# dwofk/fast-depth

Hardware: NVIDIA H100
Metric: depth-maps/sec @224x224 b64 (higher is better)
Workload: dtype f16

## Files before the change

fastdepth_b200/csrc/fd_block_tc.cu:

```cuda
#include <cuda.h>

#include <cstdio>
#include <cstdlib>
#include <cstring>
#include <new>
#include <string>

#include "fd_block_plan.h"
#include "fd_tc_common.cuh"

namespace fd {

constexpr int TC_DW_WARPS = 8;
constexpr int TC_EPI_WARPS = 8;
constexpr int TC_WARP_EPI0 = 0, TC_WARP_DW0 = TC_EPI_WARPS;
constexpr int TC_WARP_TMA = TC_DW_WARPS + TC_EPI_WARPS;
constexpr int TC_THREADS = (TC_WARP_TMA + 1) * 32;
constexpr int TC_WARP_BCAST = TC_WARP_TMA + 1;
constexpr int TC_THREADS_CL = (TC_WARP_BCAST + 1) * 32;
constexpr int TC_NCH = 2;
constexpr int TC_KBLK = 64;
constexpr int TC_A_STAGE_BYTES = 128 * 128;
constexpr int TC_MAX_IN = 6, TC_MAX_A = 6, TC_MAX_B = 16;
static_assert(TC_MAX_A >= kPlanMaxACluster && TC_MAX_A >= kPlanMaxA && TC_MAX_IN >= kPlanMaxIn && TC_MAX_B >= kPlanMaxB, "barrier arrays cover the planner's ring depths");
constexpr int TC_TRACE_N = 256;

struct TcParams {
    int n, h_in, w_in, h_out, w_out, c_in, c_out;
    int tiles_x, tiles_y;
    int items, splits;
    int kblocks;
    int cin_pad;
    int n_cta;
    int bn;
// ... 44 lines not shown
    const int split = w - (int)t * p.splits;
    uint32_t t2 = fdiv40(t, p.mg_tx);
    const int tile_x = (int)(t - t2 * (uint32_t)p.tiles_x);
    uint32_t t3 = fdiv40(t2, p.mg_ty);
    const int tile_y = (int)(t2 - t3 * (uint32_t)p.tiles_y);
    c.img0 = (int)t3 * NI; c.oy0 = tile_y * TH; c.ox0 = tile_x * TW; c.n0 = split * p.n_cta;
    return c;
}

#define TC_TRACE(row, idx)                                                                       \
    do {                                                                                         \
        if (p.trace != nullptr && blockIdx.x == 0 && (idx) < TC_TRACE_N) p.trace[(row) * TC_TRACE_N + (idx)] = clock64(); \
    } while (0)

template <typename T, int KS, int STRIDE, int NI, int TH, int TW, bool RELU6, bool HALFK = false, int CLM = 0>
__global__ void __launch_bounds__(CLM == 1 ? TC_THREADS_CL : TC_THREADS, 1)
block_tc_kernel(const __grid_constant__ CUtensorMap tm_in, const __grid_constant__ CUtensorMap tm_w,
                const __grid_constant__ CUtensorMap tm_o0, const __grid_constant__ CUtensorMap tm_o1,
                const __grid_constant__ CUtensorMap tm_o2, const __grid_constant__ CUtensorMap tm_o3, const TcParams p) {
    static_assert(NI * TH * TW == 128, "tile must hold 128 pixels");
    static_assert(NI * (TH / 4) * (TW / 4) == TC_DW_WARPS, "one 4x4 pixel block per depthwise warp");
    constexpr int PAD = (KS - 1) / 2;
    constexpr int IH = (TH - 1) * STRIDE + KS, IW = (TW - 1) * STRIDE + KS;
    constexpr int IBH = 3 * STRIDE + KS, IBW = 3 * STRIDE + KS;
    using MF = MixFma<T>;

    extern __shared__ uint8_t smem_raw[];
    const uint32_t smem_base = (smem_u32(smem_raw) + 1023u) & ~1023u;
    uint8_t* smem = smem_raw + (smem_base - smem_u32(smem_raw));
    const uint32_t a_off = 0;
    const uint32_t b_off = a_off + p.s_a * TC_A_STAGE_BYTES;
// ... 45 lines not shown
        tma_prefetch_desc(&tm_w);
        if (p.epi_tma) { tma_prefetch_desc(&tm_o0); if (p.upsample) { tma_prefetch_desc(&tm_o1); tma_prefetch_desc(&tm_o2); tma_prefetch_desc(&tm_o3); } }
    }
    if (p.head)
        for (int i = 2 * threadIdx.x; i < p.cpad_all; i += 2 * (int)blockDim.x) s_head_w2[i >> 1] = MF::pack(p.head_w[i], p.head_w[i + 1]);
    if constexpr (HALFK) {
        for (int i = threadIdx.x; i < p.s_a * (TC_A_STAGE_BYTES / 16); i += (int)blockDim.x)
            reinterpret_cast<uint4*>(smem + a_off)[i] = make_uint4(0u, 0u, 0u, 0u);
        fence_proxy_async();
    }
    pdl_launch_dependents();
    pdl_wait_prior_grid();
    if constexpr (CLM != 0) cluster_sync_all();
    else __syncthreads();

    if (warp == TC_WARP_TMA) {
        if (lane == 0) {
            Ring rin;
            int tr = 0;
            for (int u = u_first; u < u_count; u += u_stride) {
                const int w = item_of(u);
                const ItemCoord c = decode_item(p, w, NI, TH, TW);
                for (int kb = CL ? (int)crank : 0; kb < p.kblocks; kb += (int)cs, rin.next((uint32_t)p.s_in)) {
                    const uint32_t s = rin.s, ph = rin.ph;
                    mbar_wait_sleep_sel<kHint>(smem_u32(&bars->in_empty[s]), ph ^ 1u, (uint32_t)p.sleep_ns >> 2);
                    mbar_expect_tx(smem_u32(&bars->in_full[s]), (uint32_t)(p.in_stage_bytes + p.dwp_bytes));
                    tma_load_4d(smem_base + in_off + s * p.in_stage_stride, &tm_in, smem_u32(&bars->in_full[s]), kb * TC_KBLK,
                                c.ox0 * STRIDE - PAD, c.oy0 * STRIDE - PAD, c.img0);
                    bulk_load(smem_base + in_off + s * p.in_stage_stride + p.in_stage_bytes,
                              reinterpret_cast<const uint8_t*>(p.dwp) + (size_t)kb * p.dwp_bytes, (uint32_t)p.dwp_bytes,
// ... 34 lines not shown
        if (lane == 0) {
            Ring ra;
            uint32_t o = 0;
            for (int u = u_first; u < u_count; u += u_stride)
                for (int kb = 0; kb < p.kblocks; ++kb, ra.next((uint32_t)p.s_a)) {
                    if ((uint32_t)kb % cs != crank) continue;
                    mbar_wait_sel<kHint>(smem_u32(&bars->dw_done[o & 3u]), (o >> 2) & 1u);
                    ++o;
                    const uint32_t slot = smem_base + a_off + ra.s * TC_A_STAGE_BYTES, bar = smem_u32(&bars->a_full[ra.s]);
                    mbar_arrive(bar);
                    for (uint32_t peer = 0; peer < cs; ++peer)
                        if (peer != crank) bulk_copy_to_peer(mapa_u32(slot, peer), slot, (uint32_t)TC_A_STAGE_BYTES, mapa_u32(bar, peer));
                }
        }
    } else if (rwarp >= TC_WARP_DW0 && rwarp < TC_WARP_DW0 + TC_DW_WARPS) {
        constexpr int BPR = TW / 4, BPI = (TH / 4) * BPR;
        const int dwi = rwarp - TC_WARP_DW0;
        const int teams = CL ? 1 : p.dw_teams;
        const int team = teams == 2 ? dwi >> 2 : 0, member = teams == 2 ? dwi & 3 : dwi, nblk = teams;
        Ring rin, ra;
        int tr = 0;
        uint32_t own = 0;
        const bool tracer = dwi == 0 && lane == 0;
        for (int u = u_first; u < u_count; u += u_stride) {
            for (int kb = 0; kb < p.kblocks; ++kb, ra.next((uint32_t)p.s_a)) {
                if (CL && (uint32_t)kb % cs != crank) {
                    mbar_wait_sel<kHint>(smem_u32(&bars->a_empty[ra.s]), ra.ph ^ 1u);
                    continue;
                }
                const uint32_t s = rin.s, ph = rin.ph, sa = ra.s, pha = ra.ph;
                rin.next((uint32_t)p.s_in);
                if (teams == 2 && (int)(own & 1u) != team) { ++own; continue; }
                mbar_wait_sleep_sel<kHint>(smem_u32(&bars->in_full[s]), ph, (uint32_t)p.dw_sleep_ns);
                if (tracer) TC_TRACE(1, tr);
                const uint8_t* stage = smem + in_off + s * p.in_stage_stride;
                const uint8_t* prm = stage + p.in_stage_bytes;
                const f32x2 sc = *reinterpret_cast<const f32x2*>(prm + KS * KS * 128 + lane * 8);
                const f32x2 bi = *reinterpret_cast<const f32x2*>(prm + KS * KS * 128 + 256 + lane * 8);
                mbar_wait_sel<kHint>(smem_u32(&bars->a_empty[sa]), pha ^ 1u);
                uint8_t* a_s = smem + a_off + sa * TC_A_STAGE_BYTES;
                constexpr bool kDwFfma2 = KS == 3;
                uint32_t wv[(HALFK || kDwFfma2) ? 1 : KS * KS];
                if constexpr (!HALFK && !kDwFfma2) {
#pragma unroll
                    for (int i = 0; i < KS * KS; ++i) wv[i] = *reinterpret_cast<const uint32_t*>(prm + i * 128 + lane * 4);
                }
#pragma unroll 1
                for (int blk = 0; blk < nblk; ++blk) {
                const int bidx = member * nblk + blk;
                const int ni = bidx / BPI, rem = bidx % BPI, br = rem / BPR, bc = rem % BPR;
                const uint8_t* in_s = stage + (uint32_t)((ni * IH + br * 4 * STRIDE) * IW + bc * 4 * STRIDE) * 128u + lane * 4u;
                if constexpr (HALFK) {
                    static_assert(KS == 3 && STRIDE == 1, "half-K depthwise exists for the 3x3 stride-1 block only");
                    const int hl = lane & 15, hh = lane >> 4;
                    const uint8_t* in_h = in_s - lane * 4 + hl * 4 + (hh * 2 * IW) * 128;
                    const f32x2 sc2 = *reinterpret_cast<const f32x2*>(prm + KS * KS * 128 + hl * 8);
                    const f32x2 bi2 = *reinterpret_cast<const f32x2*>(prm + KS * KS * 128 + 256 + hl * 8);
                    f32x2 acc[2][4];
#pragma unroll
                    for (int a = 0; a < 2; ++a)
// ... 52 lines not shown
#pragma unroll
                            for (int ox = 0; ox < 4; ++ox)
#pragma unroll
                                for (int kx = 0; kx < KS; ++kx) ffma2(acc[oy][ox], row[ox * STRIDE + kx], wq[ky][kx]);
                            if (ky == KS - 1) {
#pragma unroll
                                for (int ox = 0; ox < 4; ++ox) {
                                    const int m = (ni * TH + br * 4 + oy) * TW + bc * 4 + ox;
                                    *reinterpret_cast<uint32_t*>(a_s + m * 128 + (((lane >> 2) ^ (m & 7)) << 4) + ((lane & 3) << 2)) =
                                        MF::template pack_act<RELU6>(ffma2_abc(acc[oy][ox], sc, bi));
                                }
                            }
                        }
                    }
                } else {
                    float acc[4][4][2];
#pragma unroll
                    for (int a = 0; a < 4; ++a)
#pragma unroll
                        for (int b = 0; b < 4; ++b) acc[a][b][0] = acc[a][b][1] = 0.f;
#pragma unroll
                    for (int iy = 0; iy < IBH; ++iy) {
                        uint32_t row[IBW];
#pragma unroll
                        for (int ix = 0; ix < IBW; ++ix) row[ix] = *reinterpret_cast<const uint32_t*>(in_s + (iy * IW + ix) * 128);
#pragma unroll
                        for (int oy = 0; oy < 4; ++oy) {
                            const int ky = iy - oy * STRIDE;
                            if (ky < 0 || ky >= KS) continue;
#pragma unroll
                            for (int ox = 0; ox < 4; ++ox)
#pragma unroll
                                for (int kx = 0; kx < KS; ++kx)
                                    MF::fma2(acc[oy][ox][0], acc[oy][ox][1], row[ox * STRIDE + kx], wv[ky * KS + kx]);
                            if (ky == KS - 1) {
#pragma unroll
                                for (int ox = 0; ox < 4; ++ox) {
                                    const int m = (ni * TH + br * 4 + oy) * TW + bc * 4 + ox;
                                    *reinterpret_cast<uint32_t*>(a_s + m * 128 + (((lane >> 2) ^ (m & 7)) << 4) + ((lane & 3) << 2)) =
                                        MF::template pack_act<RELU6>(ffma2_abc(f32x2_make(acc[oy][ox][0], acc[oy][ox][1]), sc, bi));
                                }
                            }
                        }
                    }
                }
                }
                if (tracer) TC_TRACE(2, tr);
                __syncwarp();
                if (lane == 0) mbar_arrive(smem_u32(&bars->in_empty[s]));
                fence_proxy_async();
                __syncwarp();
                if (lane == 0) mbar_arrive(CL ? smem_u32(&bars->dw_done[own & 3u]) : smem_u32(&bars->a_full[sa]));
                ++own;
                if (tracer) { TC_TRACE(3, tr); ++tr; }
            }
        }
    } else {
        const int ew = rwarp - TC_WARP_EPI0;
        const int wg = ew >> 2, wq = ew & 3;
        const int r0 = wg * 64 + wq * 16 + (lane >> 2), cq = (lane & 3) * 2;
        const bool leader = wq == 0 && lane == 0;
        const bool elected = ew == 0 && lane == 0;
        constexpr uint32_t bar_id = 1u, bar_n = 256u;
        T* __restrict__ outp = reinterpret_cast<T*>(p.out);
        const T* __restrict__ skipp = reinterpret_cast<const T*>(p.skip);
        const int n_stg = p.n_stg < 2 ? 1 : 2;
        const int nch = (p.n_cta + 63) >> 6;
        const int bn_ch = p.bn >> 6;
        const uint32_t a_lo0 = sw128_desc_lo(smem_base + a_off + (uint32_t)wg * 8192u), b_lo0 = sw128_desc_lo(smem_base + b_off);
        const uint32_t a_step = TC_A_STAGE_BYTES >> 4, b_step = (uint32_t)p.b_stage_bytes >> 4;
        Ring ra, rb;
        int tr = 0;
// ... 29 lines not shown
                        --q_left;
                    }
                }
                if (elected) TC_TRACE(4, tr);
                uint32_t sbs[TC_NCH] = {0u, 0u};
                for (int nbi = 0; nbi * bn_ch < nch; ++nbi) {
                    uint32_t sb;
                    if (p.b_resident) {
                        sb = (uint32_t)(kb * (nch / bn_ch) + nbi);
                        if (first) mbar_wait_sel<kHint>(smem_u32(&bars->b_full[sb]), 0);
                    } else {
                        sb = rb.s;
                        mbar_wait_sel<kHint>(smem_u32(&bars->b_full[sb]), rb.ph);
                        rb.next((uint32_t)p.s_b);
                    }
                    sbs[nbi] = sb;
                }
                const uint32_t a_lo = a_lo0 + ra.s * a_step;
                wgmma_fence();
#pragma unroll
                for (int j = 0; j < TC_NCH; ++j) {
                    if (j < nch) {
                        const uint32_t b_lo = b_lo0 + (bn_ch == 2 ? sbs[0] * b_step + (uint32_t)j * 512u : sbs[j] * b_step);
#pragma unroll
                        for (int k4 = 0; k4 < 4; ++k4)
                            wgmma_n64<T>(acc[j], sw128_desc(a_lo + 2u * k4), sw128_desc(b_lo + 2u * k4), (kb > 0 || k4 > 0) ? 1u : 0u);
                    }
                }
                wgmma_commit();
                wgmma_wait0();
                if (leader) {
                    const uint32_t bar_a = smem_u32(&bars->a_empty[ra.s]);
                    if constexpr (CL) { for (uint32_t r = 0; r < cs; ++r) mbar_arrive_cluster(mapa_u32(bar_a, r)); }
                    else mbar_arrive(bar_a);
                    if (!p.b_resident)
                        for (int nbi = 0; nbi * bn_ch < nch; ++nbi) {
                            const uint32_t bar_b = smem_u32(&bars->b_empty[sbs[nbi]]);
                            if constexpr (CW) { for (uint32_t r = 0; r < wmc; ++r) mbar_arrive_cluster(mapa_u32(bar_b, r)); }
                            else mbar_arrive(bar_b);
                        }
                }
                if (elected) { TC_TRACE(5, tr); ++tr; }
            }

            if (!p.head) {
                const float2* aff = s_pw_affine + c.n0;
#pragma unroll
                for (int cb = 0; cb < TC_NCH; ++cb) {
                    if (cb >= nch) break;
                    uint8_t* stg = smem + stg_off + (n_stg == 2 ? (stg_flip & 1u) * 16384u : 0u);
                    ++stg_flip;
                    if (n_stg == 1 && stg_flip > 1) {
// ... 176 lines not shown

template <typename T, int KS, int STRIDE, int NI, int TH, int TW, bool RELU6, bool HALFK = false, int CLM = 0>
static int launch_inst2(BlockTcPlan* bp, cudaStream_t st) {
    auto kern = block_tc_kernel<T, KS, STRIDE, NI, TH, TW, RELU6, HALFK, CLM>;
    constexpr bool CL = CLM != 0;
    const int csize = CLM == 1 ? bp->p.cs : bp->p.wmc;
    const int units = CLM == 1 ? bp->tiles : bp->p.items / (bp->p.wmc > 0 ? bp->p.wmc : 1);
    static PerDeviceOnce attr_set;
    int dev = -1;
    FD_CUDA_OK(cudaGetDevice(&dev));
    if (attr_set.need(dev)) {
        FD_CUDA_OK(cudaFuncSetAttribute(kern, cudaFuncAttributeMaxDynamicSharedMemorySize, 227 * 1024));
        attr_set.done(dev);
    }
    cudaLaunchConfig_t cfg{};
    cfg.gridDim = bp->grid; cfg.blockDim = dim3(CLM == 1 ? TC_THREADS_CL : TC_THREADS); cfg.dynamicSmemBytes = bp->smem_bytes; cfg.stream = st;
    cudaLaunchAttribute attr[2];
    int na = 0;
    if (CL) {
        attr[na].id = cudaLaunchAttributeClusterDimension;
        attr[na].val.clusterDim.x = (unsigned)csize; attr[na].val.clusterDim.y = 1; attr[na].val.clusterDim.z = 1;
        ++na;
    }
    if (CL && !bp->grid_final) {
        cfg.attrs = attr; cfg.numAttrs = (unsigned)na;
        cfg.gridDim = dim3((unsigned)(units * csize), 1, 1);
        int n_cl = 0;
        FD_CUDA_OK(cudaOccupancyMaxActiveClusters(&n_cl, kern, &cfg));
        if (n_cl < 1) return fail(FD_ERR_UNSUPPORTED, "cluster-mode block kernel: no cluster of this shape fits the device");
        if (n_cl > units) n_cl = units;
        bp->grid = dim3((unsigned)(n_cl * csize), 1, 1);
// ... 275 lines not shown
```

fastdepth_b200/csrc/fd_chain_tc.cu:

```cuda
#include <cuda.h>

#include <cstdio>
#include <cstdlib>
#include <cstring>
#include <new>
#include <string>
#include <vector>

#include "fd_tc_common.cuh"

namespace fd {

constexpr int CH_WORKERS = 16;
constexpr int CH_WARP_TMA = 16;
constexpr int CH_THREADS = 17 * 32;
constexpr int CH_MAX_PASS = 4;
constexpr int CH_MAX_LAYERS = 8, CH_MAX_KB = 8;
constexpr int CH_PITCH = 15, CH_ROWS = 9;
constexpr int CH_BLK = 136 * 128;
constexpr int CH_IN_BYTES = CH_ROWS * CH_PITCH * 128;
constexpr int CH_SB = 4, CH_B_STAGE = 128 * 128;
constexpr int CH_SD = 4, CH_DWP = 9 * 128 + 512;
constexpr int CH_AFF_BYTES = 512 * 8;
constexpr int CH_OFF_ACT = 1024;
constexpr int CH_OFF_B = CH_OFF_ACT + CH_MAX_KB * CH_BLK;
constexpr int CH_OFF_DWP = CH_OFF_B + CH_SB * CH_B_STAGE;
constexpr int CH_OFF_AFF = CH_OFF_DWP + CH_SD * CH_DWP;
constexpr int CH_OFF_BAR = CH_OFF_AFF + 2 * CH_AFF_BYTES;

struct ChainBarriers {
// ... 25 lines not shown
    int out_pitch;
    int sleep_ns;
    int n_zero[2];
    void* out;
    ChainLayer L[CH_MAX_LAYERS];
    unsigned long long* trace;
    unsigned char zero_slots[2][48];
};

struct ChainMaps {
    CUtensorMap in;
    CUtensorMap w[CH_MAX_LAYERS];
    CUtensorMap out[2];
};

__device__ __forceinline__ void st_cluster_u32(uint32_t cluster_addr, uint32_t v) {
    asm volatile("st.shared::cluster.b32 [%0], %1;" ::"r"(cluster_addr), "r"(v) : "memory");
}

#define CH_TRACE(row, idx)                                                                                \
    do {                                                                                                  \
        if (p.trace != nullptr && blockIdx.x == 0 && (idx) < 256) p.trace[(row) * 256 + (idx)] = clock64(); \
    } while (0)

template <typename T, bool RELU6>
__global__ void __cluster_dims__(2, 1, 1) __launch_bounds__(CH_THREADS, 1)
chain_tc_kernel(const __grid_constant__ ChainMaps maps, const __grid_constant__ ChainParams p) {
    using MF = MixFma<T>;
    extern __shared__ uint8_t smem_raw[];
    const uint32_t smem_base = (smem_u32(smem_raw) + 1023u) & ~1023u;
// ... 14 lines not shown
        mbar_init(smem_u32(&bars->halo_full), 1);
        mbar_init(smem_u32(&bars->act_free), 1);
        fence_barrier_init();
    }
    for (int i = threadIdx.x; i < (CH_OFF_B) / 16; i += CH_THREADS) reinterpret_cast<uint4*>(smem)[i] = make_uint4(0u, 0u, 0u, 0u);
    fence_proxy_async();
    if (warp == CH_WARP_TMA && lane == 0) {
        tma_prefetch_desc(&maps.in);
        tma_prefetch_desc(&maps.out[rank]);
        for (int l = 0; l < p.n_layers; ++l) tma_prefetch_desc(&maps.w[l]);
    }
    pdl_launch_dependents();
    pdl_wait_prior_grid();
    cluster_sync_all();

    if (warp == CH_WARP_TMA) {
        if (lane == 0) {
            uint32_t seq = 0;
            for (int img = cluster_id; img < p.n_img; img += n_clusters)
                for (int l = 0; l < p.n_layers; ++l) {
                    const ChainLayer& L = p.L[l];
                    for (int ps = 0; ps < L.np; ++ps)
                        for (int kb = 0; kb < L.kblocks; ++kb, ++seq) {
                            const uint32_t s = seq & (CH_SB - 1), ph = (seq / CH_SB) & 1u;
                            mbar_wait_sleep(smem_u32(&bars->b_empty[s]), ph ^ 1u, (uint32_t)p.sleep_ns);
                            if (kb == 0 && ps == 0 && img == cluster_id) CH_TRACE(10, l);
                            mbar_expect_tx(smem_u32(&bars->b_full[s]), (uint32_t)CH_B_STAGE);
                            tma_load_2d(smem_base + CH_OFF_B + s * CH_B_STAGE, &maps.w[l], smem_u32(&bars->b_full[s]), kb * 64, ps * 128);
                        }
                }
        } else if (lane == 1) {
            uint32_t dseq = 0, lseq = 0;
// ... 13 lines not shown
                        bulk_load(smem_base + CH_OFF_DWP + s * CH_DWP, reinterpret_cast<const uint8_t*>(L.dwp) + (size_t)kb * CH_DWP,
                                  (uint32_t)CH_DWP, smem_u32(&bars->dwp_full[s]));
                    }
                }
        } else if (lane == 2) {
            uint32_t it = 0;
            for (int img = cluster_id; img < p.n_img; img += n_clusters, ++it) {
                if (it > 0) mbar_wait_sleep(smem_u32(&bars->act_free), (it - 1u) & 1u, (uint32_t)p.sleep_ns);
                for (int kb = 0; kb < p.L[0].kblocks; ++kb) {
                    mbar_expect_tx(smem_u32(&bars->in_full[kb]), (uint32_t)CH_IN_BYTES);
                    tma_load_4d(smem_base + CH_OFF_ACT + kb * CH_BLK, &maps.in, smem_u32(&bars->in_full[kb]), kb * 64, 0, row_first - 1, img);
                }
            }
        }
    } else {
        const int grp = warp >> 3, wi = warp & 7;
        const bool dw_active = wi < 7;
        const int tx0 = 2 * (dw_active ? wi : 0);
        const int s0 = tx0 - 1;
        uint32_t rd_off[8];
#pragma unroll
        for (int j = 0; j < 8; ++j) rd_off[j] = ((((uint32_t)lane >> 2) ^ ((uint32_t)(s0 + j) & 7u)) << 4) + (((uint32_t)lane & 3u) << 2);
        uint32_t wr_off[2];
#pragma unroll
        for (int ox = 0; ox < 2; ++ox) wr_off[ox] = ((((uint32_t)lane >> 2) ^ ((uint32_t)(tx0 + ox) & 7u)) << 4) + (((uint32_t)lane & 3u) << 2);
        const int nzc = p.n_zero[rank] * 8;
        const uint32_t z_off = (int)threadIdx.x < nzc ? (uint32_t)p.zero_slots[rank][threadIdx.x >> 3] * 128u + ((uint32_t)threadIdx.x & 7u) * 16u : 0u;
        const int rh = (warp >> 2) & 1, ch = warp >> 3, cp = (lane & 3) * 2;
        const bool wg_leader = (warp & 3) == 0 && lane == 0;
        int e_slot[2], e_halo_slot[2], e_last_slot[2];
        bool e_valid[2], e_halo[2];
#pragma unroll
        for (int h = 0; h < 2; ++h) {
            const int m = rh * 64 + (warp & 3) * 16 + (lane >> 2) + 8 * h, e_ty = m >> 4, e_tx = m & 15;
            e_valid[h] = e_ty < rows_local && e_tx < p.w;
            e_slot[h] = (e_ty + 1) * CH_PITCH + e_tx;
            e_last_slot[h] = e_ty * CH_PITCH + e_tx;
            e_halo[h] = e_valid[h] && (rank == 0 ? e_ty == rows_local - 1 : e_ty == 0);
            e_halo_slot[h] = (rank == 0 ? 0 : (p.rows0 + 1) * CH_PITCH) + e_tx;
        }
        const uint32_t peer_act = mapa_u32(smem_base + CH_OFF_ACT, rank ^ 1u);
        const uint32_t peer_halo_full = mapa_u32(smem_u32(&bars->halo_full), rank ^ 1u);
        const uint32_t peer_mma_done = mapa_u32(smem_u32(&bars->mma_done), rank ^ 1u);
        uint32_t dseq_base = 0, lseq = 0, halo_seq = 0, it = 0, bseq = 0, a_par = 0;
        for (int img = cluster_id; img < p.n_img; img += n_clusters, ++it) {
            for (int l = 0; l < p.n_layers; ++l, ++lseq) {
                const ChainLayer& L = p.L[l];
                const bool last = l == p.n_layers - 1;
                const bool tr0 = it == 0 && warp == 0 && lane == 0, tr8 = it == 0 && warp == 8 && lane == 0;
                if (tr0) CH_TRACE(0, l);
                for (int kb = grp; kb < L.kblocks; kb += 2) {
                    uint8_t* blk = smem + CH_OFF_ACT + kb * CH_BLK;
                    if (l == 0) mbar_wait_sleep(smem_u32(&bars->in_full[kb]), it & 1u, (uint32_t)p.sleep_ns);
                    const uint32_t dseq = dseq_base + (uint32_t)kb, ds = dseq & (CH_SD - 1), dph = (dseq / CH_SD) & 1u;
                    mbar_wait(smem_u32(&bars->dwp_full[ds]), dph);
                    const uint8_t* prm = smem + CH_OFF_DWP + ds * CH_DWP;
                    const f32x2 sc = *reinterpret_cast<const f32x2*>(prm + 9 * 128 + lane * 8);
                    const f32x2 bi = *reinterpret_cast<const f32x2*>(prm + 9 * 128 + 256 + lane * 8);
                    const uint8_t* in0 = blk + s0 * 128;
                    uint32_t o[7][2];
                    if (dw_active) {
                        f32x2 acc[7][2];
#pragma unroll
                        for (int a = 0; a < 7; ++a) acc[a][0] = acc[a][1] = 0ull;
                        f32x2 wq[3][3];
#pragma unroll
                        for (int iy = 0; iy < 9; ++iy) {
                            if (iy < 3) {
#pragma unroll
                                for (int kx = 0; kx < 3; ++kx) wq[iy][kx] = MF::widen(*reinterpret_cast<const uint32_t*>(prm + (iy * 3 + kx) * 128 + lane * 4));
                            }
                            f32x2 row[4];
#pragma unroll
                            for (int ix = 0; ix < 4; ++ix) {
                                const int k = iy * CH_PITCH + ix;
                                row[ix] = MF::widen(*reinterpret_cast<const uint32_t*>(in0 + k * 128 + rd_off[k & 7]));
// ... 7 lines not shown
#pragma unroll
                                    for (int kx = 0; kx < 3; ++kx) ffma2(acc[oy][ox], row[ox + kx], wq[ky][kx]);
                            }
                        }
#pragma unroll
                        for (int oy = 0; oy < 7; ++oy)
#pragma unroll
                            for (int ox = 0; ox < 2; ++ox) o[oy][ox] = MF::template pack_act<RELU6>(ffma2_abc(acc[oy][ox], sc, bi));
                    }
                    __syncwarp();
                    if (tr0 && kb == 0) CH_TRACE(1, l);
                    if (lane == 0) mbar_arrive(smem_u32(&bars->dwp_empty[ds]));
                    asm volatile("bar.sync %0, %1;" ::"r"(1 + grp), "r"(256) : "memory");
                    if (dw_active) {
#pragma unroll
                        for (int oy = 0; oy < 7; ++oy)
#pragma unroll
                            for (int ox = 0; ox < 2; ++ox)
                                *reinterpret_cast<uint32_t*>(blk + (oy * 16 + tx0 + ox) * 128 + wr_off[ox]) = o[oy][ox];
                    }
                    fence_proxy_async();
                    __syncwarp();
                    if (lane == 0) mbar_arrive(smem_u32(&bars->a_full[kb]));
                }
                dseq_base += (uint32_t)L.kblocks;
                if (tr0) CH_TRACE(2, l);
                if (tr8) CH_TRACE(9, l);

                const uint32_t as = lseq & 1u;
                mbar_wait(smem_u32(&bars->aff_full[as]), (lseq >> 1) & 1u);
                const float2* aff = reinterpret_cast<const float2*>(smem + CH_OFF_AFF + as * CH_AFF_BYTES);
                uint32_t pk[CH_MAX_PASS][16];
#pragma unroll
                for (int ps = 0; ps < CH_MAX_PASS; ++ps) {
                    if (ps >= L.np) break;
                    const int col0 = ps * 128 + ch * 64;
                    const bool act = col0 < L.n_pad;
                    float acc[32];
#pragma unroll
                    for (int i = 0; i < 32; ++i) acc[i] = 0.f;
                    for (int kb = 0; kb < L.kblocks; ++kb, ++bseq) {
                        const uint32_t s = bseq & (CH_SB - 1), ph = (bseq / CH_SB) & 1u;
                        mbar_wait(smem_u32(&bars->a_full[kb]), (a_par >> kb) & 1u);
                        mbar_wait(smem_u32(&bars->b_full[s]), ph);
                        if (tr0 && kb == 0 && ps == 0) CH_TRACE(7, l);
                        if (act) {
                            const uint32_t a_lo = sw128_desc_lo(smem_base + CH_OFF_ACT + (uint32_t)kb * CH_BLK + (uint32_t)rh * 8192u);
                            const uint32_t b_lo = sw128_desc_lo(smem_base + CH_OFF_B + s * CH_B_STAGE + (uint32_t)ch * 8192u);
                            wgmma_fence();
#pragma unroll
                            for (int k4 = 0; k4 < 4; ++k4)
                                wgmma_n64<T>(acc, sw128_desc(a_lo + 2u * k4), sw128_desc(b_lo + 2u * k4), (kb > 0 || k4 > 0) ? 1u : 0u);
                            wgmma_commit();
                            wgmma_wait0();
                        }
                        if (wg_leader) mbar_arrive(smem_u32(&bars->b_empty[s]));
                    }
#pragma unroll
                    for (int i = 0; i < 8; ++i) {
                        const int c = col0 + i * 8 + cp;
                        const bool ok = act && col0 + i * 8 < L.n_pad;
                        const float4 af = ok ? *reinterpret_cast<const float4*>(aff + c) : make_float4(0.f, 0.f, 0.f, 0.f);
#pragma unroll
                        for (int h = 0; h < 2; ++h)
                            pk[ps][8 * h + i] = MF::template pack_act<RELU6>(ffma2_abc(f32x2_make(acc[4 * i + 2 * h], acc[4 * i + 2 * h + 1]),
                                                                                        f32x2_make(af.x, af.y), f32x2_make(af.z, af.w)));
                    }
                }
                for (int kb = 0; kb < L.kblocks; ++kb) a_par ^= 1u << kb;
                if (tr0) CH_TRACE(8, l);
                asm volatile("bar.sync %0, %1;" ::"r"(3), "r"(CH_WORKERS * 32) : "memory");
                if (!last) {
                    if (threadIdx.x == 0) mbar_arrive_cluster(peer_mma_done);
                    mbar_wait_cluster(smem_u32(&bars->mma_done), halo_seq & 1u, 0u);
                }
                if (tr0) CH_TRACE(3, l);
#pragma unroll
                for (int ps = 0; ps < CH_MAX_PASS; ++ps) {
                    if (ps >= L.np) break;
                    const int col0 = ps * 128 + ch * 64;
                    if (col0 >= L.n_pad) continue;
                    const uint32_t boff = (uint32_t)(col0 >> 6) * CH_BLK;
#pragma unroll
                    for (int h = 0; h < 2; ++h) {
                        const int w_slot = last ? e_last_slot[h] : e_slot[h];
#pragma unroll
                        for (int i = 0; i < 8; ++i) {
                            if (col0 + i * 8 >= L.n_pad) break;
                            if (e_valid[h])
                                *reinterpret_cast<uint32_t*>(smem + CH_OFF_ACT + boff + w_slot * 128 + (((uint32_t)i ^ ((uint32_t)w_slot & 7u)) << 4) + cp * 2) =
                                    pk[ps][8 * h + i];
                            if (e_halo[h] && !last)
                                st_cluster_u32(peer_act + boff + (uint32_t)e_halo_slot[h] * 128u + (((uint32_t)i ^ ((uint32_t)e_halo_slot[h] & 7u)) << 4) + cp * 2,
                                               pk[ps][8 * h + i]);
                        }
                    }
                }
                if (tr0) CH_TRACE(4, l);
                if (!last) {
                    if ((int)threadIdx.x < nzc) {
                        const int kbn = p.L[l + 1].kblocks;
                        for (int kb = 0; kb < kbn; ++kb)
                            *reinterpret_cast<uint4*>(smem + CH_OFF_ACT + kb * CH_BLK + z_off) = make_uint4(0u, 0u, 0u, 0u);
                    }
                }
                fence_proxy_async();
                __syncwarp();
                if (lane == 0) mbar_arrive(smem_u32(&bars->aff_empty[as]));
                asm volatile("bar.sync %0, %1;" ::"r"(3), "r"(CH_WORKERS * 32) : "memory");
                if (!last && threadIdx.x == 0) mbar_arrive_cluster(peer_halo_full);
                if (tr0) CH_TRACE(5, l);
                if (!last) { mbar_wait_cluster(smem_u32(&bars->halo_full), halo_seq & 1u, 0u); ++halo_seq; }
                if (last && threadIdx.x == 0) {
                    for (int kb = 0; kb < (L.c_out + 63) / 64; ++kb)
                        tma_store_4d(&maps.out[rank], smem_base + CH_OFF_ACT + kb * CH_BLK, kb * 64, 0, row_first, img);
                    bulk_commit_group();
                    bulk_wait_read0();
                    mbar_arrive(smem_u32(&bars->act_free));
                }
                if (tr0) CH_TRACE(6, l);
            }
        }
        if (threadIdx.x == 0) bulk_wait_all();
    }

// ... 195 lines not shown
```

fastdepth_b200/csrc/fd_tc_common.cuh:

```cuda
#pragma once
#include <cuda.h>
#include <cstdio>

#include "fd_common.cuh"

namespace fd {

__device__ __forceinline__ uint32_t smem_u32(const void* p) { return (uint32_t)__cvta_generic_to_shared(p); }

__device__ __forceinline__ void mbar_init(uint32_t bar, uint32_t count) {
    asm volatile("mbarrier.init.shared::cta.b64 [%0], %1;" ::"r"(bar), "r"(count));
}
__device__ __forceinline__ void mbar_arrive(uint32_t bar) {
    asm volatile("mbarrier.arrive.shared::cta.b64 _, [%0];" ::"r"(bar) : "memory");
}
__device__ __forceinline__ void mbar_expect_tx(uint32_t bar, uint32_t bytes) {
    asm volatile("mbarrier.arrive.expect_tx.shared::cta.b64 _, [%0], %1;" ::"r"(bar), "r"(bytes) : "memory");
}
#ifdef FD_TC_WATCHDOG
__device__ __forceinline__ void mbar_wait(uint32_t bar, uint32_t parity) {
    const long long t0 = clock64();
    for (;;) {
        uint32_t ok;
        asm volatile("{\n\t.reg .pred p;\n\tmbarrier.try_wait.parity.shared::cta.b64 p, [%1], %2;\n\tselp.u32 %0, 1, 0, p;\n\t}" : "=r"(ok) : "r"(bar), "r"(parity) : "memory");
// ... 87 lines not shown
__device__ __forceinline__ void bulk_commit_group() { asm volatile("cp.async.bulk.commit_group;" ::: "memory"); }
__device__ __forceinline__ void bulk_wait_read0() { asm volatile("cp.async.bulk.wait_group.read 0;" ::: "memory"); }
__device__ __forceinline__ void bulk_wait_read1() { asm volatile("cp.async.bulk.wait_group.read 1;" ::: "memory"); }
__device__ __forceinline__ void bulk_wait_all() { asm volatile("cp.async.bulk.wait_group 0;" ::: "memory"); }
__device__ __forceinline__ void tma_prefetch_desc(const CUtensorMap* map) {
    asm volatile("prefetch.tensormap [%0];" ::"l"(map) : "memory");
}

constexpr uint32_t kSw128DescHi = (1024u >> 4) | (1u << 30);
__device__ __forceinline__ uint32_t sw128_desc_lo(uint32_t saddr) { return ((saddr >> 4) & 0x3FFFu) | (1u << 16); }
__device__ __forceinline__ uint64_t sw128_desc(uint32_t lo) { return ((uint64_t)kSw128DescHi << 32) | lo; }
__device__ __forceinline__ void wgmma_fence() { asm volatile("wgmma.fence.sync.aligned;" ::: "memory"); }
__device__ __forceinline__ void wgmma_commit() { asm volatile("wgmma.commit_group.sync.aligned;" ::: "memory"); }
__device__ __forceinline__ void wgmma_wait0() { asm volatile("wgmma.wait_group.sync.aligned 0;" ::: "memory"); }
__device__ __forceinline__ void wgmma_wait1() { asm volatile("wgmma.wait_group.sync.aligned 1;" ::: "memory"); }
#define FD_WGMMA_N64(TY)                                                                                                        \
    asm volatile("{\n\t.reg .pred p;\n\tsetp.ne.b32 p, %34, 0;\n\t"                                                          \
                 "wgmma.mma_async.sync.aligned.m64n64k16.f32." TY "." TY " "                                                   \
                 "{%0,%1,%2,%3,%4,%5,%6,%7,%8,%9,%10,%11,%12,%13,%14,%15,%16,%17,%18,%19,%20,%21,%22,%23,%24,%25,%26,%27,%28,"  \
                 "%29,%30,%31}, %32, %33, p, 1, 1, 0, 0;\n\t}"                                                                  \
                 : "+f"(d[0]), "+f"(d[1]), "+f"(d[2]), "+f"(d[3]), "+f"(d[4]), "+f"(d[5]), "+f"(d[6]), "+f"(d[7]), "+f"(d[8]),    \
                   "+f"(d[9]), "+f"(d[10]), "+f"(d[11]), "+f"(d[12]), "+f"(d[13]), "+f"(d[14]), "+f"(d[15]), "+f"(d[16]),         \
                   "+f"(d[17]), "+f"(d[18]), "+f"(d[19]), "+f"(d[20]), "+f"(d[21]), "+f"(d[22]), "+f"(d[23]), "+f"(d[24]),        \
                   "+f"(d[25]), "+f"(d[26]), "+f"(d[27]), "+f"(d[28]), "+f"(d[29]), "+f"(d[30]), "+f"(d[31])                      \
                 : "l"(a), "l"(b), "r"(acc))
#define FD_WGMMA_N32(TY)                                                                                                        \
    asm volatile("{\n\t.reg .pred p;\n\tsetp.ne.b32 p, %18, 0;\n\t"                                                          \
                 "wgmma.mma_async.sync.aligned.m64n32k16.f32." TY "." TY " "                                                   \
                 "{%0,%1,%2,%3,%4,%5,%6,%7,%8,%9,%10,%11,%12,%13,%14,%15}, %16, %17, p, 1, 1, 0, 0;\n\t}"                      \
                 : "+f"(d[0]), "+f"(d[1]), "+f"(d[2]), "+f"(d[3]), "+f"(d[4]), "+f"(d[5]), "+f"(d[6]), "+f"(d[7]), "+f"(d[8]),    \
// ... 177 lines not shown
```

Measured before the change: 52090.

## Rebalance registers with setmaxnreg and overlap chain wgmma with B-slot release

Both kernels are padded to whole warpgroups so the producer warps can give up registers with setmaxnreg.dec while the depthwise, epilogue and worker warps raise their limit. Several per-thread precomputed offsets in the chain kernel are now recomputed on demand to lower register pressure. Depthwise accumulation switches to packed f32x2 with pre-widened operands. The chain GEMM loop now waits on the previous wgmma group instead of all groups and frees B stages one step late, so loads can overlap the MMA. In exchange there are extra idle producer warps, more address arithmetic, and a risk of spills or a wrong register budget.

```diff
diff --git a/fastdepth_b200/csrc/fd_block_tc.cu b/fastdepth_b200/csrc/fd_block_tc.cu
--- a/fastdepth_b200/csrc/fd_block_tc.cu
+++ b/fastdepth_b200/csrc/fd_block_tc.cu
@@ -15,9 +15,11 @@
 constexpr int TC_EPI_WARPS = 8;
 constexpr int TC_WARP_EPI0 = 0, TC_WARP_DW0 = TC_EPI_WARPS;
 constexpr int TC_WARP_TMA = TC_DW_WARPS + TC_EPI_WARPS;
-constexpr int TC_THREADS = (TC_WARP_TMA + 1) * 32;
 constexpr int TC_WARP_BCAST = TC_WARP_TMA + 1;
-constexpr int TC_THREADS_CL = (TC_WARP_BCAST + 1) * 32;
+constexpr int TC_THREADS = (TC_WARP_TMA + 4) * 32;
+constexpr uint32_t TC_REG_PRODUCER = 24, TC_REG_DW = 112, TC_REG_EPI = 112;
+static_assert(4 * 32 * TC_REG_PRODUCER + TC_DW_WARPS * 32 * TC_REG_DW + TC_EPI_WARPS * 32 * TC_REG_EPI <= TC_THREADS * launch_regs(TC_THREADS),
+              "register budgets exceed the launch allocation");
 constexpr int TC_NCH = 2;
 constexpr int TC_KBLK = 64;
 constexpr int TC_A_STAGE_BYTES = 128 * 128;
@@ -92,7 +94,7 @@
     } while (0)
 
 template <typename T, int KS, int STRIDE, int NI, int TH, int TW, bool RELU6, bool HALFK = false, int CLM = 0>
-__global__ void __launch_bounds__(CLM == 1 ? TC_THREADS_CL : TC_THREADS, 1)
+__global__ void __launch_bounds__(TC_THREADS, 1)
 block_tc_kernel(const __grid_constant__ CUtensorMap tm_in, const __grid_constant__ CUtensorMap tm_w,
                 const __grid_constant__ CUtensorMap tm_o0, const __grid_constant__ CUtensorMap tm_o1,
                 const __grid_constant__ CUtensorMap tm_o2, const __grid_constant__ CUtensorMap tm_o3, const TcParams p) {
@@ -168,6 +170,7 @@
     if constexpr (CLM != 0) cluster_sync_all();
     else __syncthreads();
 
+    if (warp >= TC_WARP_TMA) setmaxnreg_dec<TC_REG_PRODUCER>();
     if (warp == TC_WARP_TMA) {
         if (lane == 0) {
             Ring rin;
@@ -232,6 +235,7 @@
                 }
         }
     } else if (rwarp >= TC_WARP_DW0 && rwarp < TC_WARP_DW0 + TC_DW_WARPS) {
+        setmaxnreg_inc<TC_REG_DW>();
         constexpr int BPR = TW / 4, BPI = (TH / 4) * BPR;
         const int dwi = rwarp - TC_WARP_DW0;
         const int teams = CL ? 1 : p.dw_teams;
@@ -258,10 +262,10 @@
                 mbar_wait_sel<kHint>(smem_u32(&bars->a_empty[sa]), pha ^ 1u);
                 uint8_t* a_s = smem + a_off + sa * TC_A_STAGE_BYTES;
                 constexpr bool kDwFfma2 = KS == 3;
-                uint32_t wv[(HALFK || kDwFfma2) ? 1 : KS * KS];
+                f32x2 wv[(HALFK || kDwFfma2) ? 1 : KS * KS];
                 if constexpr (!HALFK && !kDwFfma2) {
 #pragma unroll
-                    for (int i = 0; i < KS * KS; ++i) wv[i] = *reinterpret_cast<const uint32_t*>(prm + i * 128 + lane * 4);
+                    for (int i = 0; i < KS * KS; ++i) wv[i] = MF::widen(*reinterpret_cast<const uint32_t*>(prm + i * 128 + lane * 4));
                 }
 #pragma unroll 1
                 for (int blk = 0; blk < nblk; ++blk) {
@@ -344,16 +348,16 @@
                         }
                     }
                 } else {
-                    float acc[4][4][2];
+                    f32x2 acc[4][4];
 #pragma unroll
                     for (int a = 0; a < 4; ++a)
 #pragma unroll
-                        for (int b = 0; b < 4; ++b) acc[a][b][0] = acc[a][b][1] = 0.f;
+                        for (int b = 0; b < 4; ++b) acc[a][b] = 0ull;
 #pragma unroll
                     for (int iy = 0; iy < IBH; ++iy) {
-                        uint32_t row[IBW];
-#pragma unroll
-                        for (int ix = 0; ix < IBW; ++ix) row[ix] = *reinterpret_cast<const uint32_t*>(in_s + (iy * IW + ix) * 128);
+                        f32x2 row[IBW];
+#pragma unroll
+                        for (int ix = 0; ix < IBW; ++ix) row[ix] = MF::widen(*reinterpret_cast<const uint32_t*>(in_s + (iy * IW + ix) * 128));
 #pragma unroll
                         for (int oy = 0; oy < 4; ++oy) {
                             const int ky = iy - oy * STRIDE;
@@ -361,14 +365,13 @@
 #pragma unroll
                             for (int ox = 0; ox < 4; ++ox)
 #pragma unroll
-                                for (int kx = 0; kx < KS; ++kx)
-                                    MF::fma2(acc[oy][ox][0], acc[oy][ox][1], row[ox * STRIDE + kx], wv[ky * KS + kx]);
+                                for (int kx = 0; kx < KS; ++kx) ffma2(acc[oy][ox], row[ox * STRIDE + kx], wv[ky * KS + kx]);
                             if (ky == KS - 1) {
 #pragma unroll
                                 for (int ox = 0; ox < 4; ++ox) {
                                     const int m = (ni * TH + br * 4 + oy) * TW + bc * 4 + ox;
                                     *reinterpret_cast<uint32_t*>(a_s + m * 128 + (((lane >> 2) ^ (m & 7)) << 4) + ((lane & 3) << 2)) =
-                                        MF::template pack_act<RELU6>(ffma2_abc(f32x2_make(acc[oy][ox][0], acc[oy][ox][1]), sc, bi));
+                                        MF::template pack_act<RELU6>(ffma2_abc(acc[oy][ox], sc, bi));
                                 }
                             }
                         }
@@ -385,7 +388,8 @@
                 if (tracer) { TC_TRACE(3, tr); ++tr; }
             }
         }
-    } else {
+    } else if (rwarp < TC_WARP_EPI0 + TC_EPI_WARPS) {
+        setmaxnreg_inc<TC_REG_EPI>();
         const int ew = rwarp - TC_WARP_EPI0;
         const int wg = ew >> 2, wq = ew & 3;
         const int r0 = wg * 64 + wq * 16 + (lane >> 2), cq = (lane & 3) * 2;
@@ -445,7 +449,7 @@
                         mbar_wait_sel<kHint>(smem_u32(&bars->b_full[sb]), rb.ph);
                         rb.next((uint32_t)p.s_b);
                     }
-                    sbs[nbi] = sb;
+                    if (nbi == 0) sbs[0] = sb; else sbs[1] = sb;
                 }
                 const uint32_t a_lo = a_lo0 + ra.s * a_step;
                 wgmma_fence();
@@ -466,7 +470,7 @@
                     else mbar_arrive(bar_a);
                     if (!p.b_resident)
                         for (int nbi = 0; nbi * bn_ch < nch; ++nbi) {
-                            const uint32_t bar_b = smem_u32(&bars->b_empty[sbs[nbi]]);
+                            const uint32_t bar_b = smem_u32(&bars->b_empty[nbi == 0 ? sbs[0] : sbs[1]]);
                             if constexpr (CW) { for (uint32_t r = 0; r < wmc; ++r) mbar_arrive_cluster(mapa_u32(bar_b, r)); }
                             else mbar_arrive(bar_b);
                         }
@@ -673,7 +677,7 @@
         attr_set.done(dev);
     }
     cudaLaunchConfig_t cfg{};
-    cfg.gridDim = bp->grid; cfg.blockDim = dim3(CLM == 1 ? TC_THREADS_CL : TC_THREADS); cfg.dynamicSmemBytes = bp->smem_bytes; cfg.stream = st;
+    cfg.gridDim = bp->grid; cfg.blockDim = dim3(TC_THREADS); cfg.dynamicSmemBytes = bp->smem_bytes; cfg.stream = st;
     cudaLaunchAttribute attr[2];
     int na = 0;
     if (CL) {
diff --git a/fastdepth_b200/csrc/fd_chain_tc.cu b/fastdepth_b200/csrc/fd_chain_tc.cu
--- a/fastdepth_b200/csrc/fd_chain_tc.cu
+++ b/fastdepth_b200/csrc/fd_chain_tc.cu
@@ -13,7 +13,10 @@
 
 constexpr int CH_WORKERS = 16;
 constexpr int CH_WARP_TMA = 16;
-constexpr int CH_THREADS = 17 * 32;
+constexpr int CH_THREADS = 20 * 32;
+constexpr uint32_t CH_REG_PRODUCER = 24, CH_REG_WORKER = 112;
+static_assert(4 * 32 * CH_REG_PRODUCER + CH_WORKERS * 32 * CH_REG_WORKER <= CH_THREADS * launch_regs(CH_THREADS),
+              "register budgets exceed the launch allocation");
 constexpr int CH_MAX_PASS = 4;
 constexpr int CH_MAX_LAYERS = 8, CH_MAX_KB = 8;
 constexpr int CH_PITCH = 15, CH_ROWS = 9;
@@ -69,6 +72,8 @@
     CUtensorMap out[2];
 };
 
+__device__ __forceinline__ uint32_t tid_opaque() { uint32_t t; asm volatile("mov.u32 %0, %%tid.x;" : "=r"(t)); return t; }
+
 __device__ __forceinline__ void st_cluster_u32(uint32_t cluster_addr, uint32_t v) {
     asm volatile("st.shared::cluster.b32 [%0], %1;" ::"r"(cluster_addr), "r"(v) : "memory");
 }
@@ -113,8 +118,10 @@
     pdl_wait_prior_grid();
     cluster_sync_all();
 
-    if (warp == CH_WARP_TMA) {
-        if (lane == 0) {
+    if (warp >= CH_WORKERS) {
+        setmaxnreg_dec<CH_REG_PRODUCER>();
+        if (warp != CH_WARP_TMA) {
+        } else if (lane == 0) {
             uint32_t seq = 0;
             for (int img = cluster_id; img < p.n_img; img += n_clusters)
                 for (int l = 0; l < p.n_layers; ++l) {
@@ -158,34 +165,10 @@
             }
         }
     } else {
-        const int grp = warp >> 3, wi = warp & 7;
-        const bool dw_active = wi < 7;
-        const int tx0 = 2 * (dw_active ? wi : 0);
-        const int s0 = tx0 - 1;
-        uint32_t rd_off[8];
-#pragma unroll
-        for (int j = 0; j < 8; ++j) rd_off[j] = ((((uint32_t)lane >> 2) ^ ((uint32_t)(s0 + j) & 7u)) << 4) + (((uint32_t)lane & 3u) << 2);
-        uint32_t wr_off[2];
-#pragma unroll
-        for (int ox = 0; ox < 2; ++ox) wr_off[ox] = ((((uint32_t)lane >> 2) ^ ((uint32_t)(tx0 + ox) & 7u)) << 4) + (((uint32_t)lane & 3u) << 2);
-        const int nzc = p.n_zero[rank] * 8;
-        const uint32_t z_off = (int)threadIdx.x < nzc ? (uint32_t)p.zero_slots[rank][threadIdx.x >> 3] * 128u + ((uint32_t)threadIdx.x & 7u) * 16u : 0u;
+        setmaxnreg_inc<CH_REG_WORKER>();
+        const int grp = warp >> 3;
         const int rh = (warp >> 2) & 1, ch = warp >> 3, cp = (lane & 3) * 2;
         const bool wg_leader = (warp & 3) == 0 && lane == 0;
-        int e_slot[2], e_halo_slot[2], e_last_slot[2];
-        bool e_valid[2], e_halo[2];
-#pragma unroll
-        for (int h = 0; h < 2; ++h) {
-            const int m = rh * 64 + (warp & 3) * 16 + (lane >> 2) + 8 * h, e_ty = m >> 4, e_tx = m & 15;
-            e_valid[h] = e_ty < rows_local && e_tx < p.w;
-            e_slot[h] = (e_ty + 1) * CH_PITCH + e_tx;
-            e_last_slot[h] = e_ty * CH_PITCH + e_tx;
-            e_halo[h] = e_valid[h] && (rank == 0 ? e_ty == rows_local - 1 : e_ty == 0);
-            e_halo_slot[h] = (rank == 0 ? 0 : (p.rows0 + 1) * CH_PITCH) + e_tx;
-        }
-        const uint32_t peer_act = mapa_u32(smem_base + CH_OFF_ACT, rank ^ 1u);
-        const uint32_t peer_halo_full = mapa_u32(smem_u32(&bars->halo_full), rank ^ 1u);
-        const uint32_t peer_mma_done = mapa_u32(smem_u32(&bars->mma_done), rank ^ 1u);
         uint32_t dseq_base = 0, lseq = 0, halo_seq = 0, it = 0, bseq = 0, a_par = 0;
         for (int img = cluster_id; img < p.n_img; img += n_clusters, ++it) {
             for (int l = 0; l < p.n_layers; ++l, ++lseq) {
@@ -194,6 +177,10 @@
                 const bool tr0 = it == 0 && warp == 0 && lane == 0, tr8 = it == 0 && warp == 8 && lane == 0;
                 if (tr0) CH_TRACE(0, l);
                 for (int kb = grp; kb < L.kblocks; kb += 2) {
+                    const int wi = (int)(tid_opaque() >> 5) & 7;
+                    const bool dw_active = wi < 7;
+                    const int tx0 = 2 * (dw_active ? wi : 0);
+                    const int s0 = tx0 - 1;
                     uint8_t* blk = smem + CH_OFF_ACT + kb * CH_BLK;
                     if (l == 0) mbar_wait_sleep(smem_u32(&bars->in_full[kb]), it & 1u, (uint32_t)p.sleep_ns);
                     const uint32_t dseq = dseq_base + (uint32_t)kb, ds = dseq & (CH_SD - 1), dph = (dseq / CH_SD) & 1u;
@@ -204,6 +191,9 @@
                     const uint8_t* in0 = blk + s0 * 128;
                     uint32_t o[7][2];
                     if (dw_active) {
+                        uint32_t rd_off[8];
+#pragma unroll
+                        for (int j = 0; j < 8; ++j) rd_off[j] = ((((uint32_t)lane >> 2) ^ ((uint32_t)(s0 + j) & 7u)) << 4) + (((uint32_t)lane & 3u) << 2);
                         f32x2 acc[7][2];
 #pragma unroll
                         for (int a = 0; a < 7; ++a) acc[a][0] = acc[a][1] = 0ull;
@@ -241,10 +231,11 @@
                     asm volatile("bar.sync %0, %1;" ::"r"(1 + grp), "r"(256) : "memory");
                     if (dw_active) {
 #pragma unroll
-                        for (int oy = 0; oy < 7; ++oy)
-#pragma unroll
-                            for (int ox = 0; ox < 2; ++ox)
-                                *reinterpret_cast<uint32_t*>(blk + (oy * 16 + tx0 + ox) * 128 + wr_off[ox]) = o[oy][ox];
+                        for (int ox = 0; ox < 2; ++ox) {
+                            const uint32_t wr_off = ((((uint32_t)lane >> 2) ^ ((uint32_t)(tx0 + ox) & 7u)) << 4) + (((uint32_t)lane & 3u) << 2);
+#pragma unroll
+                            for (int oy = 0; oy < 7; ++oy) *reinterpret_cast<uint32_t*>(blk + (oy * 16 + tx0 + ox) * 128 + wr_off) = o[oy][ox];
+                        }
                     }
                     fence_proxy_async();
                     __syncwarp();
@@ -266,12 +257,12 @@
                     float acc[32];
 #pragma unroll
                     for (int i = 0; i < 32; ++i) acc[i] = 0.f;
-                    for (int kb = 0; kb < L.kblocks; ++kb, ++bseq) {
-                        const uint32_t s = bseq & (CH_SB - 1), ph = (bseq / CH_SB) & 1u;
-                        mbar_wait(smem_u32(&bars->a_full[kb]), (a_par >> kb) & 1u);
-                        mbar_wait(smem_u32(&bars->b_full[s]), ph);
-                        if (tr0 && kb == 0 && ps == 0) CH_TRACE(7, l);
-                        if (act) {
+                    if (act) {
+                        for (int kb = 0; kb < L.kblocks; ++kb, ++bseq) {
+                            const uint32_t s = bseq & (CH_SB - 1), ph = (bseq / CH_SB) & 1u;
+                            mbar_wait(smem_u32(&bars->a_full[kb]), (a_par >> kb) & 1u);
+                            mbar_wait(smem_u32(&bars->b_full[s]), ph);
+                            if (tr0 && kb == 0 && ps == 0) CH_TRACE(7, l);
                             const uint32_t a_lo = sw128_desc_lo(smem_base + CH_OFF_ACT + (uint32_t)kb * CH_BLK + (uint32_t)rh * 8192u);
                             const uint32_t b_lo = sw128_desc_lo(smem_base + CH_OFF_B + s * CH_B_STAGE + (uint32_t)ch * 8192u);
                             wgmma_fence();
@@ -279,9 +270,18 @@
                             for (int k4 = 0; k4 < 4; ++k4)
                                 wgmma_n64<T>(acc, sw128_desc(a_lo + 2u * k4), sw128_desc(b_lo + 2u * k4), (kb > 0 || k4 > 0) ? 1u : 0u);
                             wgmma_commit();
-                            wgmma_wait0();
+                            wgmma_wait1();
+                            if (kb > 0 && wg_leader) mbar_arrive(smem_u32(&bars->b_empty[(bseq - 1u) & (CH_SB - 1)]));
                         }
-                        if (wg_leader) mbar_arrive(smem_u32(&bars->b_empty[s]));
+                        wgmma_wait0();
+                        if (wg_leader) mbar_arrive(smem_u32(&bars->b_empty[(bseq - 1u) & (CH_SB - 1)]));
+                    } else {
+                        for (int kb = 0; kb < L.kblocks; ++kb, ++bseq) {
+                            const uint32_t s = bseq & (CH_SB - 1), ph = (bseq / CH_SB) & 1u;
+                            mbar_wait(smem_u32(&bars->a_full[kb]), (a_par >> kb) & 1u);
+                            mbar_wait(smem_u32(&bars->b_full[s]), ph);
+                            if (wg_leader) mbar_arrive(smem_u32(&bars->b_empty[s]));
+                        }
                     }
 #pragma unroll
                     for (int i = 0; i < 8; ++i) {
@@ -298,34 +298,42 @@
                 if (tr0) CH_TRACE(8, l);
                 asm volatile("bar.sync %0, %1;" ::"r"(3), "r"(CH_WORKERS * 32) : "memory");
                 if (!last) {
-                    if (threadIdx.x == 0) mbar_arrive_cluster(peer_mma_done);
+                    if (threadIdx.x == 0) mbar_arrive_cluster(mapa_u32(smem_u32(&bars->mma_done), rank ^ 1u));
                     mbar_wait_cluster(smem_u32(&bars->mma_done), halo_seq & 1u, 0u);
                 }
                 if (tr0) CH_TRACE(3, l);
 #pragma unroll
-                for (int ps = 0; ps < CH_MAX_PASS; ++ps) {
-                    if (ps >= L.np) break;
-                    const int col0 = ps * 128 + ch * 64;
-                    if (col0 >= L.n_pad) continue;
-                    const uint32_t boff = (uint32_t)(col0 >> 6) * CH_BLK;
-#pragma unroll
-                    for (int h = 0; h < 2; ++h) {
-                        const int w_slot = last ? e_last_slot[h] : e_slot[h];
+                for (int h = 0; h < 2; ++h) {
+                    const uint32_t t = tid_opaque();
+                    const int m = (int)((t >> 5) & 7u) * 16 + (int)((t & 31u) >> 2) + 8 * h;
+                    const int e_ty = m >> 4, e_tx = m & 15;
+                    const bool e_valid = e_ty < rows_local && e_tx < p.w;
+                    const int w_slot = (last ? e_ty : e_ty + 1) * CH_PITCH + e_tx;
+                    const bool e_halo = !last && e_valid && (rank == 0 ? e_ty == rows_local - 1 : e_ty == 0);
+                    const uint32_t e_halo_slot = (uint32_t)((rank == 0 ? 0 : (p.rows0 + 1) * CH_PITCH) + e_tx);
+#pragma unroll
+                    for (int ps = 0; ps < CH_MAX_PASS; ++ps) {
+                        if (ps >= L.np) break;
+                        const int col0 = ps * 128 + ch * 64;
+                        if (col0 >= L.n_pad) continue;
+                        const uint32_t boff = (uint32_t)(col0 >> 6) * CH_BLK;
 #pragma unroll
                         for (int i = 0; i < 8; ++i) {
                             if (col0 + i * 8 >= L.n_pad) break;
-                            if (e_valid[h])
+                            if (e_valid)
                                 *reinterpret_cast<uint32_t*>(smem + CH_OFF_ACT + boff + w_slot * 128 + (((uint32_t)i ^ ((uint32_t)w_slot & 7u)) << 4) + cp * 2) =
                                     pk[ps][8 * h + i];
-                            if (e_halo[h] && !last)
-                                st_cluster_u32(peer_act + boff + (uint32_t)e_halo_slot[h] * 128u + (((uint32_t)i ^ ((uint32_t)e_halo_slot[h] & 7u)) << 4) + cp * 2,
+                            if (e_halo)
+                                st_cluster_u32(mapa_u32(smem_base + CH_OFF_ACT, rank ^ 1u) + boff + e_halo_slot * 128u + (((uint32_t)i ^ (e_halo_slot & 7u)) << 4) + cp * 2,
                                                pk[ps][8 * h + i]);
                         }
                     }
                 }
                 if (tr0) CH_TRACE(4, l);
                 if (!last) {
-                    if ((int)threadIdx.x < nzc) {
+                    const uint32_t t = tid_opaque();
+                    if ((int)t < p.n_zero[rank] * 8) {
+                        const uint32_t z_off = (uint32_t)p.zero_slots[rank][t >> 3] * 128u + (t & 7u) * 16u;
                         const int kbn = p.L[l + 1].kblocks;
                         for (int kb = 0; kb < kbn; ++kb)
                             *reinterpret_cast<uint4*>(smem + CH_OFF_ACT + kb * CH_BLK + z_off) = make_uint4(0u, 0u, 0u, 0u);
@@ -335,7 +343,7 @@
                 __syncwarp();
                 if (lane == 0) mbar_arrive(smem_u32(&bars->aff_empty[as]));
                 asm volatile("bar.sync %0, %1;" ::"r"(3), "r"(CH_WORKERS * 32) : "memory");
-                if (!last && threadIdx.x == 0) mbar_arrive_cluster(peer_halo_full);
+                if (!last && threadIdx.x == 0) mbar_arrive_cluster(mapa_u32(smem_u32(&bars->halo_full), rank ^ 1u));
                 if (tr0) CH_TRACE(5, l);
                 if (!last) { mbar_wait_cluster(smem_u32(&bars->halo_full), halo_seq & 1u, 0u); ++halo_seq; }
                 if (last && threadIdx.x == 0) {
diff --git a/fastdepth_b200/csrc/fd_tc_common.cuh b/fastdepth_b200/csrc/fd_tc_common.cuh
--- a/fastdepth_b200/csrc/fd_tc_common.cuh
+++ b/fastdepth_b200/csrc/fd_tc_common.cuh
@@ -125,6 +125,9 @@
 __device__ __forceinline__ void wgmma_commit() { asm volatile("wgmma.commit_group.sync.aligned;" ::: "memory"); }
 __device__ __forceinline__ void wgmma_wait0() { asm volatile("wgmma.wait_group.sync.aligned 0;" ::: "memory"); }
 __device__ __forceinline__ void wgmma_wait1() { asm volatile("wgmma.wait_group.sync.aligned 1;" ::: "memory"); }
+constexpr int launch_regs(int threads) { return 65536 / threads / 8 * 8; }
+template <uint32_t N> __device__ __forceinline__ void setmaxnreg_dec() { asm volatile("setmaxnreg.dec.sync.aligned.u32 %0;" ::"n"(N)); }
+template <uint32_t N> __device__ __forceinline__ void setmaxnreg_inc() { asm volatile("setmaxnreg.inc.sync.aligned.u32 %0;" ::"n"(N)); }
 #define FD_WGMMA_N64(TY)                                                                                                        \
     asm volatile("{\n\t.reg .pred p;\n\tsetp.ne.b32 p, %34, 0;\n\t"                                                          \
                  "wgmma.mma_async.sync.aligned.m64n64k16.f32." TY "." TY " "                                                   \
```

Result: faster. 60020 (median of 6 runs) (+15.2%).
